# solislemuslab/BayesianNetworkRegression.jl

Hardware: NVIDIA B200
Metric: gibbs_iters_per_sec_all_chains (higher is better)
Workload: dtype f64

## Files before the change

### bayesiannetworkregression.jl_b200/csrc/bnr_linalg.cu

```cuda
#include <cstdio>
#include <cstdlib>
#include <cstring>
#include <cuda.h>
#include "bnr_engine.cuh"
#include "bnr_kernels.h"

namespace bnr {

__device__ __forceinline__ void dmma884(double& c0, double& c1, double a, double b) {
  asm volatile("mma.sync.aligned.m8n8k4.row.col.f64.f64.f64.f64 {%0,%1}, {%2}, {%3}, {%0,%1};\n"
               : "+d"(c0), "+d"(c1) : "d"(a), "d"(b));
}
__device__ __forceinline__ double neg_bits(double x) {
  return __longlong_as_double(__double_as_longlong(x) ^ (long long)0x8000000000000000ull);
}
__device__ __forceinline__ void cp_async_commit() { asm volatile("cp.async.commit_group;\n" ::); }
template <int N>
__device__ __forceinline__ void cp_async_wait() { asm volatile("cp.async.wait_group %0;\n" ::"n"(N)); }
__device__ __forceinline__ void cp_async16(void* smem, const void* gmem) {
  const unsigned sa = (unsigned)__cvta_generic_to_shared(smem);
  asm volatile("cp.async.cg.shared.global [%0], [%1], 16;\n" ::"r"(sa), "l"(gmem));
}

__device__ __forceinline__ unsigned smem_u32(const void* p) { return (unsigned)__cvta_generic_to_shared(p); }
// ... 1297 lines not shown
#pragma unroll
      for (int nf = 0; nf < 4; ++nf) {
        if (nf < nfv) {
#pragma unroll
          for (int mf = 0; mf < 4; ++mf) dmma884(acc[mf][nf][0], acc[mf][nf][1], af[mf], bf[nf]);
        }
      }
    }
  }
  cp_async_wait<0>();
#pragma unroll
  for (int mf = 0; mf < 4; ++mf) {
    const int mm = m0 + wm * 32 + mf * 8 + lr;
#pragma unroll
    for (int nf = 0; nf < 4; ++nf) {
      const int nn = n0 + wn * 32 + nf * 8 + 2 * lk;
      if (mm < M) {
        if (nn < N) o[(size_t)nn * ldout + mm] = acc[mf][nf][0];
        if (nn + 1 < N) o[(size_t)(nn + 1) * ldout + mm] = acc[mf][nf][1];
      }
    }
  }
}

__global__ void k_splitk_reduce(const double* __restrict__ ws, double* __restrict__ out, size_t count, int splits) {
  const size_t i = (size_t)blockIdx.x * blockDim.x + threadIdx.x;
  if (i >= count) return;
  double s = 0.0;
  for (int z = 0; z < splits; ++z) s += ws[(size_t)z * count + i];
  out[i] = s;
}

static int x_times_splits(const Dims& d, int trans) {
  const int M = trans ? d.qp : d.np, K = trans ? d.np : d.qp;
  const int tiles = ((M + XM_BM - 1) / XM_BM) * ((d.C_total + XM_BN - 1) / XM_BN);
  int ks = (2 * 148 + tiles - 1) / tiles;
  const int kmax = K / (4 * XM_BK) > 0 ? K / (4 * XM_BK) : 1;
  if (ks > kmax) ks = kmax;
  if (ks > 64) ks = 64;
  if (ks < 1) ks = 1;
  return ks;
}

size_t x_times_workspace_doubles(const Dims& d) {
  const int a = x_times_splits(d, 0), b = x_times_splits(d, 1);
  const size_t wa = (size_t)a * d.C_total * d.np, wb = (size_t)b * d.C_total * d.qp;
  return wa > wb ? wa : wb;
}

void launch_x_times(const Engine& e, int trans, const double* in, double* out, double* ws, cudaStream_t s) {
  const Dims& d = e.d;
  const int M = trans ? d.qp : d.np, K = trans ? d.np : d.qp, N = d.C;
  const int ldin = trans ? d.np : d.qp, ldout = trans ? d.qp : d.np;
  const int ks = x_times_splits(d, trans);
  const int kper = ((K + ks - 1) / ks + XM_BK - 1) / XM_BK * XM_BK;
  dim3 grid((M + XM_BM - 1) / XM_BM, (N + XM_BN - 1) / XM_BN, ks);
  double* dst = ks == 1 ? out : ws;
  ++g_launches;
  if (trans) k_xmma<1><<<grid, 256, XMMA_SMEM, s>>>(e.X, d.np, M, K, N, in, ldin, dst, ldout, kper);
  else k_xmma<0><<<grid, 256, XMMA_SMEM, s>>>(e.X, d.np, M, K, N, in, ldin, dst, ldout, kper);
  if (ks > 1) {
    const size_t count = (size_t)N * ldout;
    ++g_launches; k_splitk_reduce<<<(unsigned)((count + 255) / 256), 256, 0, s>>>(ws, out, count, ks);
  }
}

__global__ void k_gram_i8(const __grid_constant__ CUtensorMap tmA, const __grid_constant__ CUtensorMap tmB,
                          const double* __restrict__ rscale, double* __restrict__ G, int np, int nvalid, int nkb);
extern const size_t GI_SMEM_BYTES;

void linalg_setup() {
  cudaFuncSetAttribute(k_xmma<0>, cudaFuncAttributeMaxDynamicSharedMemorySize, (int)XMMA_SMEM);
  cudaFuncSetAttribute(k_xmma<1>, cudaFuncAttributeMaxDynamicSharedMemorySize, (int)XMMA_SMEM);
  cudaFuncSetAttribute(k_gram_syrk, cudaFuncAttributeMaxDynamicSharedMemorySize, (int)SYRK_SMEM);
  cudaFuncSetAttribute(k_gram_i8, cudaFuncAttributeMaxDynamicSharedMemorySize, (int)GI_SMEM_BYTES);
  cudaFuncSetAttribute(k_chol_update, cudaFuncAttributeMaxDynamicSharedMemorySize, (int)SYRK_SMEM);
  cudaFuncSetAttribute(k_trsm_dmma, cudaFuncAttributeMaxDynamicSharedMemorySize, (int)SYRK_SMEM);
  cudaFuncSetAttribute(k_potf2_inv, cudaFuncAttributeMaxDynamicSharedMemorySize, (int)POTF2_SMEM);
  cudaFuncSetAttribute(k_bwd_stream, cudaFuncAttributeMaxDynamicSharedMemorySize, 227 * 1024);
  cudaFuncSetAttribute(k_bwd_cluster, cudaFuncAttributeMaxDynamicSharedMemorySize, 227 * 1024);
  cudaFuncSetAttribute(k_small_tile<1, 4>, cudaFuncAttributeMaxDynamicSharedMemorySize, (int)small_tile_smem(32));
  cudaFuncSetAttribute(k_small_tile<2, 4>, cudaFuncAttributeMaxDynamicSharedMemorySize, (int)small_tile_smem(32));
  cudaFuncSetAttribute(k_small_tile<1, 2>, cudaFuncAttributeMaxDynamicSharedMemorySize, (int)small_tile_smem(16));
  cudaFuncSetAttribute(k_small_tile<2, 2>, cudaFuncAttributeMaxDynamicSharedMemorySize, (int)small_tile_smem(16));
  cudaFuncSetAttribute(k_small_tile<1, 8>, cudaFuncAttributeMaxDynamicSharedMemorySize, (int)small_tile_smem(64));
  cudaFuncSetAttribute(k_small_tile<2, 8>, cudaFuncAttributeMaxDynamicSharedMemorySize, (int)small_tile_smem(64));
}

typedef CUresult (*TmapEncodeFn)(CUtensorMap*, CUtensorMapDataType, cuuint32_t, void*, const cuuint64_t*, const cuuint64_t*,
                                 const cuuint32_t*, const cuuint32_t*, CUtensorMapInterleave, CUtensorMapSwizzle,
                                 CUtensorMapL2promotion, CUtensorMapFloatOOBfill);
static TmapEncodeFn g_tmap_encode = nullptr;
bool tmap_setup() {
  if (g_tmap_encode) return true;
  void* fn = nullptr;
  cudaDriverEntryPointQueryResult qr;
  if (cudaGetDriverEntryPoint("cuTensorMapEncodeTiled", &fn, cudaEnableDefault, &qr) != cudaSuccess ||
      qr != cudaDriverEntryPointSuccess || !fn)
    return false;
  g_tmap_encode = (TmapEncodeFn)fn;
  return true;
}
static CUresult encode_map(CUtensorMap* m, const double* base, uint64_t rows, uint64_t krows, uint64_t ld, uint32_t box_rows,
                           uint32_t box_k) {
  memset(m, 0, sizeof(*m));
  const cuuint64_t dims[2] = {rows, krows};
  const cuuint64_t strides[1] = {ld * sizeof(double)};
  const cuuint32_t box[2] = {box_rows, box_k};
  const cuuint32_t estr[2] = {1, 1};
  if (!tmap_setup()) return CUDA_ERROR_NOT_SUPPORTED;
  return g_tmap_encode(m, CU_TENSOR_MAP_DATA_TYPE_FLOAT64, 2, const_cast<double*>(base), dims, strides, box, estr,
                       CU_TENSOR_MAP_INTERLEAVE_NONE, CU_TENSOR_MAP_SWIZZLE_NONE, CU_TENSOR_MAP_L2_PROMOTION_L2_256B,
                       CU_TENSOR_MAP_FLOAT_OOB_FILL_NONE);
}
static CUtensorMap make_map(const double* base, uint64_t rows, uint64_t krows, uint64_t ld, uint32_t box_rows,
                            uint32_t box_k = SY_BK) {
  CUtensorMap m;
  const CUresult r = encode_map(&m, base, rows, krows, ld, box_rows, box_k);
  if (r != CUDA_SUCCESS) {
    fprintf(stderr, "[bnr] cuTensorMapEncodeTiled failed (%d) for a %llu x %llu operand, box %u x %d\n", (int)r,
            (unsigned long long)rows, (unsigned long long)krows, box_rows, (int)box_k);
    abort();
  }
  return m;
}
bool tmaps_check(const Engine& e) {
  const Dims& d = e.d;
  const uint64_t N = d.gdim, C = d.C, T = d.gdim / SY_BT;
  CUtensorMap m;
  bool ok = true;
  if (d.gmode != 2) ok = ok && encode_map(&m, e.X, d.np, d.qp, d.np, SY_LDS, SY_BK) == CUDA_SUCCESS;
  for (uint32_t box : {(uint32_t)SY_LDS, (uint32_t)(SY_BT / 2 + 4), (uint32_t)(SY_BT / 4 + 4)})
    ok = ok && encode_map(&m, e.G, N, N * C, N, box, SY_BK) == CUDA_SUCCESS;
  ok = ok && encode_map(&m, e.Linv, SY_BT, SY_BT * T * C, SY_BT, SY_LDS, SY_BK) == CUDA_SUCCESS;
  ok = ok && encode_map(&m, e.G, N, N * C, N, SY_BT, BW_COLS) == CUDA_SUCCESS;
  ok = ok && encode_map(&m, e.Linv, SY_BT, SY_BT * T * C, SY_BT, SY_BT, BW_COLS) == CUDA_SUCCESS;
  return ok;
}

int syrk_splits(const Dims& d, int C) {
  const int T = d.np / SY_BT, tiles = T * (T + 1) / 2, nk = d.qp / SY_BK;
  if (const char* ov = getenv("BNR_SYRK_SPLITS")) {
    int s = atoi(ov);
    if (s > nk / 8) s = nk / 8;
    return s < 1 ? 1 : (s > SYRK_MAX_SPLITS ? SYRK_MAX_SPLITS : s);
  }
  if (tiles * C >= 148) return 1;
  int s = (4 * 148 + tiles * C - 1) / (tiles * C);
  if (s > nk / 24) s = nk / 24;
  if (s > SYRK_MAX_SPLITS) s = SYRK_MAX_SPLITS;
  return s < 1 ? 1 : s;
}

#ifndef BNR_GI_BK
#define BNR_GI_BK 64
#endif
#ifndef BNR_GI_STAGES
#define BNR_GI_STAGES 2
#endif
constexpr int GI_S = 7;
constexpr int GI_BM = 128, GI_BN = 64;
constexpr int GI_BK = BNR_GI_BK;
constexpr int GI_STAGES = BNR_GI_STAGES;
constexpr int GI_A_PLANE = GI_BM * GI_BK, GI_B_PLANE = GI_BN * GI_BK;
constexpr int GI_STAGE_BYTES = GI_S * (GI_A_PLANE + GI_B_PLANE);
constexpr size_t GI_SMEM = (size_t)GI_STAGES * GI_STAGE_BYTES + 1024 + 256;
const size_t GI_SMEM_BYTES = GI_SMEM;
constexpr int GI_THREADS = 192;
static_assert(GI_BK == 32 || GI_BK == 64 || GI_BK == 128, "k-block = swizzle width");
static_assert(GI_S * GI_BN <= 512, "accumulators exceed tensor memory");

__device__ __forceinline__ unsigned long long gi_desc(unsigned saddr) {
  constexpr unsigned long long layout = GI_BK == 128 ? 2ull : (GI_BK == 64 ? 4ull : 6ull);
  return (unsigned long long)((saddr & 0x3FFFF) >> 4) | (1ull << 16) | ((unsigned long long)((GI_BK * 8) >> 4) << 32) |
         (1ull << 46) | (layout << 61);
}
__host__ __device__ constexpr unsigned gi_idesc(int n) {
  return (2u << 4) | (1u << 7) | (1u << 10) | ((unsigned)(n >> 3) << 17) | ((unsigned)(GI_BM >> 4) << 24);
}

__device__ __forceinline__ void tma_load_3d(void* smem_dst, const CUtensorMap* tm, int x, int y, int z, unsigned long long* bar) {
  asm volatile("cp.async.bulk.tensor.3d.shared::cluster.global.tile.mbarrier::complete_tx::bytes [%0], [%1, {%2, %3, %4}], [%5];\n" ::"r"(
                   smem_u32(smem_dst)), "l"((unsigned long long)tm), "r"(x), "r"(y), "r"(z), "r"(smem_u32(bar)) : "memory");
}
__device__ __forceinline__ void umma_i8(unsigned tmem_d, unsigned long long adesc, unsigned long long bdesc, unsigned idesc,
                                        bool acc) {
  asm volatile("{\n.reg .pred p;\nsetp.ne.b32 p, %4, 0;\ntcgen05.mma.cta_group::1.kind::i8 [%0], %1, %2, %3, p;\n}\n" ::"r"(tmem_d),
               "l"(adesc), "l"(bdesc), "r"(idesc), "r"((int)acc));
}
__device__ __forceinline__ void umma_commit(unsigned long long* bar) {
  asm volatile("tcgen05.commit.cta_group::1.mbarrier::arrive::one.shared::cluster.b64 [%0];\n" ::"r"(smem_u32(bar)) : "memory");
}
__device__ __forceinline__ void tmem_ld8(unsigned taddr, int (&r)[8]) {
  asm volatile("tcgen05.ld.sync.aligned.32x32b.x8.b32 {%0,%1,%2,%3,%4,%5,%6,%7}, [%8];\n"
               : "=r"(r[0]), "=r"(r[1]), "=r"(r[2]), "=r"(r[3]), "=r"(r[4]), "=r"(r[5]), "=r"(r[6]), "=r"(r[7]) : "r"(taddr));
}

constexpr int GS_ROWS = 16, GS_CB = 4, GS_THREADS = 256, GS_TK = 512;
constexpr int GS_TKP = GS_TK + GS_TK / 8;
__device__ __forceinline__ int gs_tidx(int kk) { return kk + 2 * (kk >> 4); }

__device__ __forceinline__ void gs_roots(double (*sq)[GS_TKP], const double* __restrict__ S, int qp, int q, int ncb, int t0) {
  for (int id = threadIdx.x; id < GS_CB * GS_TK; id += GS_THREADS) {
    const int cb = id / GS_TK, kk = id % GS_TK, k = t0 + kk;
    sq[cb][gs_tidx(kk)] = cb < ncb && k < q ? sqrt(S[(size_t)cb * qp + k]) : 0.0;
  }
}

__device__ __forceinline__ void gs_load_x(double (&x)[16], const double* __restrict__ X, int np, int q, int row, int k0) {
  const bool full = k0 + 16 <= q;
#pragma unroll
  for (int j = 0; j < 16; ++j) x[j] = full || k0 + j < q ? X[row + (size_t)np * (k0 + j)] : 0.0;
}

__global__ void __launch_bounds__(GS_THREADS, 2) k_gram_slice(const double* __restrict__ X, const double* __restrict__ S,
                                                            int np, int q, int qp, int C, signed char* __restrict__ planes,
                                                            double* __restrict__ rscale) {
  __shared__ __align__(16) double sq[GS_CB][GS_TKP];
  __shared__ double red[GS_THREADS / 32][GS_CB][GS_ROWS];
  __shared__ double2 scl[GS_CB][GS_ROWS];
  const int lane = threadIdx.x & 31, warp = threadIdx.x >> 5, rr = lane & 15, h = lane >> 4;
  const int r0 = blockIdx.x * GS_ROWS, row = r0 + rr, c0 = blockIdx.y * GS_CB;
  const int ncb = C - c0 < GS_CB ? C - c0 : GS_CB;
  const double* Sb = S + (size_t)c0 * qp;
  constexpr int NW = GS_THREADS / 32, BPW = GS_TK / 32 / NW;
  double x[16];

  double m[GS_CB];
#pragma unroll
  for (int cb = 0; cb < GS_CB; ++cb) m[cb] = 0.0;
  for (int t0 = 0; t0 < q; t0 += GS_TK) {
    __syncthreads();
    gs_roots(sq, Sb, qp, q, ncb, t0);
    __syncthreads();
#pragma unroll
    for (int i = 0; i < BPW; ++i) {
      const int kk = 32 * (warp + NW * i) + 16 * h;
      if (t0 + kk >= q) continue;
      gs_load_x(x, X, np, q, row, t0 + kk);
#pragma unroll
      for (int cb = 0; cb < GS_CB; ++cb) {
        if (cb >= ncb) break;
#pragma unroll
        for (int j = 0; j < 16; j += 2) {
          const double2 s2 = *reinterpret_cast<const double2*>(&sq[cb][gs_tidx(kk + j)]);
          m[cb] = fmax(m[cb], fabs(x[j] * s2.x));
          m[cb] = fmax(m[cb], fabs(x[j + 1] * s2.y));
        }
      }
    }
  }
#pragma unroll
  for (int cb = 0; cb < GS_CB; ++cb) {
    const double o = __shfl_xor_sync(0xffffffffu, m[cb], 16);
    if (h == 0) red[warp][cb][rr] = fmax(m[cb], o);
  }
  __syncthreads();
  if (threadIdx.x < GS_CB * GS_ROWS) {
    const int cb = threadIdx.x / GS_ROWS, i = threadIdx.x % GS_ROWS;
    double mx = 0.0;
#pragma unroll
    for (int w = 0; w < NW; ++w) mx = fmax(mx, red[w][cb][i]);
    int p = 0;
    if (mx > 0.0) {
      p = 54 - ilogb(mx);
      if (ldexp(mx, p) > 126.0 * 0x1p48) --p;
    }
    if (cb < ncb) rscale[(size_t)(c0 + cb) * np + r0 + i] = ldexp(1.0, -p);
    const int p1 = p > 1000 ? 1000 : p;
    scl[cb][i] = make_double2(ldexp(1.0, p1), ldexp(1.0, p - p1));
  }

#if defined(GS_LAB_NO_STORES)
  unsigned sink = 0;
#endif
  for (int t0 = 0; t0 < qp; t0 += GS_TK) {
    __syncthreads();
    gs_roots(sq, Sb, qp, q, ncb, t0);
    __syncthreads();
#pragma unroll 1
    for (int i = 0; i < BPW; ++i) {
      const int kk = 32 * (warp + NW * i) + 16 * h;
      if (t0 + kk >= qp) continue;
      gs_load_x(x, X, np, q, row, t0 + kk);
#pragma unroll 1
      for (int cb = 0; cb < ncb; ++cb) {
        const double2 sc = scl[cb][rr];
        uint4 w[GI_S];
#pragma unroll
        for (int g = 0; g < 4; ++g) {
          unsigned lo[4], hi[4];
#pragma unroll
          for (int b = 0; b < 4; ++b) {
            const int j = 4 * g + b;
#if defined(GS_LAB_NO_DIGITS)
            lo[b] = __double2loint(x[j]) + j; hi[b] = __double2hiint(x[j]) + cb;
#else
            const double sqk = sq[cb][gs_tidx(kk + j)];
            const unsigned long long M = (unsigned long long)__double2ll_rn(x[j] * sqk * sc.x * sc.y) + 0x808080808080ull;
            lo[b] = (unsigned)M; hi[b] = (unsigned)(M >> 32);
#endif
          }
          const unsigned a0 = __byte_perm(lo[0], lo[1], 0x5140), a1 = __byte_perm(lo[0], lo[1], 0x7362);
          const unsigned a2 = __byte_perm(lo[2], lo[3], 0x5140), a3 = __byte_perm(lo[2], lo[3], 0x7362);
          const unsigned b0 = __byte_perm(hi[0], hi[1], 0x5140), b1 = __byte_perm(hi[0], hi[1], 0x7362);
          const unsigned b2 = __byte_perm(hi[2], hi[3], 0x5140), b3 = __byte_perm(hi[2], hi[3], 0x7362);
          const unsigned v[GI_S] = {__byte_perm(b1, b3, 0x5410), __byte_perm(b0, b2, 0x7632) ^ 0x80808080u,
                                    __byte_perm(b0, b2, 0x5410) ^ 0x80808080u, __byte_perm(a1, a3, 0x7632) ^ 0x80808080u,
                                    __byte_perm(a1, a3, 0x5410) ^ 0x80808080u, __byte_perm(a0, a2, 0x7632) ^ 0x80808080u,
                                    __byte_perm(a0, a2, 0x5410) ^ 0x80808080u};
#pragma unroll
          for (int s = 0; s < GI_S; ++s) (&w[s].x)[g] = v[s];
        }
        signed char* out = planes + ((size_t)(c0 + cb) * GI_S * np + row) * qp + t0 + kk;
#pragma unroll
        for (int s = 0; s < GI_S; ++s) {
#if defined(GS_LAB_NO_STORES)
          sink ^= w[s].x ^ w[s].y ^ w[s].z ^ w[s].w;
#else
          *reinterpret_cast<uint4*>(out + (size_t)s * np * qp) = w[s];
#endif
        }
      }
    }
  }
#if defined(GS_LAB_NO_STORES)
  if (sink == 0x9e3779b9u) planes[0] = 1;
#endif
}

__global__ void __launch_bounds__(GI_THREADS, 1)
k_gram_i8(const __grid_constant__ CUtensorMap tmA, const __grid_constant__ CUtensorMap tmB,
          const double* __restrict__ rscale, double* __restrict__ G, int np, int nvalid, int nkb) {
  extern __shared__ __align__(1024) unsigned char gsm_raw[];
  unsigned char* gsm = reinterpret_cast<unsigned char*>(((size_t)gsm_raw + 1023) & ~(size_t)1023);
  unsigned long long* full = reinterpret_cast<unsigned long long*>(gsm + (size_t)GI_STAGES * GI_STAGE_BYTES);
  unsigned long long* empty = full + GI_STAGES;
  unsigned long long* accf = empty + GI_STAGES;
  unsigned* tmem_slot = reinterpret_cast<unsigned*>(accf + 1);
  const int tid = threadIdx.x, lane = tid & 31, warp = tid >> 5;
  const int c = blockIdx.y;
  int ib = 0;
  while (2 * (ib + 1) * (ib + 2) / 2 <= (int)blockIdx.x) ++ib;
  const int jb = (int)blockIdx.x - ib * (ib + 1);
  const int i0 = ib * GI_BM, j0 = jb * GI_BN;
  const bool diag_block = (j0 / GI_BM) == ib;
  int rows_st = GI_BM;
  if (!diag_block) {
    int nfv = (nvalid - i0 + 7) / 8;
    if (nfv <= 0) return;
    rows_st = (nfv < 4 ? 4 : nfv) * 8;
  }
  if (tid == 0) {
    for (int s = 0; s < GI_STAGES; ++s) { mbar_init(&full[s], 1); mbar_init(&empty[s], 1); }
    mbar_init(accf, 1);
    asm volatile("fence.mbarrier_init.release.cluster;\n" ::: "memory");
  }
  if (warp == 0) {
    asm volatile("tcgen05.alloc.cta_group::1.sync.aligned.shared::cta.b32 [%0], 512;\n" ::"r"(smem_u32(tmem_slot)));
    asm volatile("tcgen05.relinquish_alloc_permit.cta_group::1.sync.aligned;\n");
  }
  asm volatile("tcgen05.fence::before_thread_sync;\n" ::: "memory");
  __syncthreads();
  asm volatile("tcgen05.fence::after_thread_sync;\n" ::: "memory");
  const unsigned tmem = *tmem_slot;

  if (warp == 4 && lane == 0) {
#if defined(GI_LAB_MMA_ONLY)
    for (int kb = 0; kb < GI_STAGES && kb < nkb; ++kb) {
#else
    for (int kb = 0; kb < nkb; ++kb) {
#endif
      const int st = kb % GI_STAGES;
      mbar_wait(&empty[st], ((kb / GI_STAGES) & 1) ^ 1);
      unsigned char* sa = gsm + (size_t)st * GI_STAGE_BYTES;
      mbar_expect_tx(&full[st], GI_STAGE_BYTES);
      tma_load_3d(sa, &tmA, kb * GI_BK, i0, c * GI_S, &full[st]);
      tma_load_3d(sa + GI_S * GI_A_PLANE, &tmB, kb * GI_BK, j0, c * GI_S, &full[st]);
    }
  } else if (warp == 5 && lane == 0) {
    for (int kb = 0; kb < nkb; ++kb) {
      const int st = kb % GI_STAGES;
#if defined(GI_LAB_MMA_ONLY)
      if (kb < GI_STAGES) mbar_wait(&full[st], 0);
#else
      mbar_wait(&full[st], (kb / GI_STAGES) & 1);
#endif
      asm volatile("tcgen05.fence::after_thread_sync;\n" ::: "memory");
#if defined(GI_LAB_LOADS_ONLY)
      umma_commit(&empty[st]);
      continue;
#endif
      const unsigned sa = smem_u32(gsm + (size_t)st * GI_STAGE_BYTES), sb = sa + GI_S * GI_A_PLANE;
#pragma unroll
      for (int kk = 0; kk < GI_BK / 32; ++kk) {
#pragma unroll
        for (int s = 0; s < GI_S; ++s) {
          const unsigned long long ad = gi_desc(sa + s * GI_A_PLANE + kk * 32);
#pragma unroll
          for (int t0 = 0; t0 < GI_S - s; t0 += 4) {
            const int nt = GI_S - s - t0 < 4 ? GI_S - s - t0 : 4;
            umma_i8(tmem + (unsigned)((s + t0) * GI_BN), ad, gi_desc(sb + t0 * GI_B_PLANE + kk * 32), gi_idesc(nt * GI_BN),
                    kb > 0 || kk > 0 || s > 0);
          }
        }
      }
      umma_commit(&empty[st]);
    }
    umma_commit(accf);
  } else if (warp < 4) {
    mbar_wait(accf, 0);
    asm volatile("tcgen05.fence::after_thread_sync;\n" ::: "memory");
    const int r = warp * 32 + lane, i = i0 + r;
    const double ri = rscale[(size_t)c * np + i] * 0x1p96;
    double* Gc = G + (size_t)c * np * np;
    const unsigned trow = tmem + ((unsigned)(warp * 32) << 16);
    for (int j8 = 0; j8 < GI_BN; j8 += 8) {
      int acc[GI_S][8];
#pragma unroll
      for (int g = 0; g < GI_S; ++g) tmem_ld8(trow + (unsigned)(g * GI_BN + j8), acc[g]);
      asm volatile("tcgen05.wait::ld.sync.aligned;\n" ::: "memory");
#pragma unroll
      for (int jj = 0; jj < 8; ++jj) {
        const int j = j0 + j8 + jj;
        double v = (double)acc[GI_S - 1][jj];
#pragma unroll
        for (int g = GI_S - 2; g >= 0; --g) v = (double)acc[g][jj] + v * 0x1p-8;
        v = v * ri * rscale[(size_t)c * np + j];
        if (i == j) v += 1.0;
        if (r < rows_st && (i >> 3) >= (j >> 3)) Gc[(size_t)j * np + i] = v;
      }
    }
  }
  asm volatile("tcgen05.fence::before_thread_sync;\n" ::: "memory");
  __syncthreads();
  if (warp == 0) {
    asm volatile("tcgen05.fence::after_thread_sync;\n" ::: "memory");
    asm volatile("tcgen05.dealloc.cta_group::1.sync.aligned.b32 %0, 512;\n" ::"r"(tmem));
  }
}

bool gram_i8_selected(const Dims& d) { return d.gmode == 1 && d.qp >= GRAM_I8_QP_MIN && d.qp <= GRAM_I8_QP_MAX; }

size_t gram_i8_plane_bytes(const Dims& d) { return (size_t)GI_S * d.np * d.qp; }

static CUresult encode_planes_map(CUtensorMap* m, const signed char* planes, const Dims& d, int C, uint32_t box_rows) {
  memset(m, 0, sizeof(*m));
  const cuuint64_t dims[3] = {(cuuint64_t)d.qp, (cuuint64_t)d.np, (cuuint64_t)GI_S * C};
  const cuuint64_t strides[2] = {(cuuint64_t)d.qp, (cuuint64_t)d.qp * d.np};
  const cuuint32_t box[3] = {(cuuint32_t)GI_BK, box_rows, (cuuint32_t)GI_S};
  const cuuint32_t estr[3] = {1, 1, 1};
  const CUtensorMapSwizzle sw = GI_BK == 128 ? CU_TENSOR_MAP_SWIZZLE_128B
                                             : (GI_BK == 64 ? CU_TENSOR_MAP_SWIZZLE_64B : CU_TENSOR_MAP_SWIZZLE_32B);
  if (!tmap_setup()) return CUDA_ERROR_NOT_SUPPORTED;
  return g_tmap_encode(m, CU_TENSOR_MAP_DATA_TYPE_UINT8, 3, const_cast<signed char*>(planes), dims, strides, box, estr,
                       CU_TENSOR_MAP_INTERLEAVE_NONE, sw, CU_TENSOR_MAP_L2_PROMOTION_L2_256B, CU_TENSOR_MAP_FLOAT_OOB_FILL_NONE);
}

static void launch_gram_i8_products(const Engine& e, cudaStream_t s) {
  const Dims& d = e.d;
  CUtensorMap tmA, tmB;
  if (encode_planes_map(&tmA, e.gram_planes, d, d.C, GI_BM) != CUDA_SUCCESS ||
      encode_planes_map(&tmB, e.gram_planes, d, d.C, GI_BN) != CUDA_SUCCESS) {
    fprintf(stderr, "[bnr] cuTensorMapEncodeTiled failed for the Gram digit planes (%d x %d)\n", d.np, d.qp);
    abort();
  }
  const int T = d.np / GI_BM;
  ++g_launches; k_gram_i8<<<dim3(T * (T + 1), d.C), GI_THREADS, GI_SMEM, s>>>(tmA, tmB, e.gram_rscale, e.G, d.np, d.n,
                                                                             (d.qp + GI_BK - 1) / GI_BK);
}

static void launch_gram_slice(const Engine& e, cudaStream_t s) {
  const Dims& d = e.d;
  ++g_launches; k_gram_slice<<<dim3(d.np / GS_ROWS, (d.C + GS_CB - 1) / GS_CB), GS_THREADS, 0, s>>>(
      e.X, e.S, d.np, d.q, d.qp, d.C, e.gram_planes, e.gram_rscale);
}

static void launch_gram_i8(const Engine& e, cudaStream_t s) {
  launch_gram_slice(e, s);
  launch_gram_i8_products(e, s);
}

void launch_syrk_G(const Engine& e, cudaStream_t s) {
  const Dims& d = e.d;
  if (gram_i8_selected(d)) {
    launch_gram_i8(e, s);
    if (e.aux.G_copy) {
      dim3 g2(d.np, d.C);
      ++g_launches; k_copy_sym<<<g2, 256, 0, s>>>(e.G, (size_t)d.np * d.np, d.np, e.aux.G_copy);
    }
    return;
  }
  const int T = d.np / SY_BT;
  const int nk = d.qp / SY_BK;
  const int ns = e.syrk_ws ? e.syrk_ws_cap + 1 : 1;
  const int nk_split = (nk + ns - 1) / ns;
#if defined(SYRK_LAB_ONLY_DIAG)
  dim3 grid(d.C, ns, T);
#elif defined(SYRK_LAB_ONLY_OFFDIAG)
  dim3 grid(d.C, ns, T * (T - 1) / 2);
#else
  dim3 grid(d.C, ns, T * (T + 1) / 2);
#endif
  const size_t gs = (size_t)d.np * d.np;
  const CUtensorMap tmX = make_map(e.X, d.np, d.qp, d.np, SY_LDS);
  ++g_launches; k_gram_syrk<<<grid, SY_THREADS, SYRK_SMEM, s>>>(tmX, e.S, (size_t)d.qp, e.G, gs, d.np, d.n, nk, 1.0,
                                                            nk_split, e.syrk_ws, e.syrk_ws_cap);
  if (ns > 1) {
    dim3 g2(T * (T + 1) / 2 * 8, d.C);
    ++g_launches; k_syrk_splitk_reduce<<<g2, 256, 0, s>>>(e.G, gs, d.np, e.syrk_ws, e.syrk_ws_cap, ns - 1);
  }
  if (e.aux.G_copy) {
    dim3 g2(d.np, d.C);
    ++g_launches; k_copy_sym<<<g2, 256, 0, s>>>(e.G, gs, d.np, e.aux.G_copy);
  }
}

void launch_xtx(const Dims& d, const double* XT, const double* ones, double* XtX, cudaStream_t s) {
  const int T = d.qp / SY_BT;
  dim3 grid(1, 1, T * (T + 1) / 2);
  const CUtensorMap tmXT = make_map(XT, d.qp, d.np, d.qp, SY_LDS);
  ++g_launches; k_gram_syrk<<<grid, SY_THREADS, SYRK_SMEM, s>>>(tmXT, ones, 0, XtX, 0, d.qp, d.q, d.np / SY_BK, 0.0,
                                                            d.np / SY_BK, nullptr, 0);
}

__global__ void __launch_bounds__(256) k_build_P(Engine e) {
  const Dims& d = e.d;
  if (blockIdx.x < blockIdx.y) return;
  const int c = blockIdx.z, N = d.qp;
  const int i = blockIdx.x * 32 + threadIdx.x;
  const double it2 = 1.0 / e.tau2[c];
  double* Gc = e.G + (size_t)c * N * N;
#pragma unroll
  for (int jj = 0; jj < 4; ++jj) {
    const int j = blockIdx.y * 32 + threadIdx.y * 4 + jj;
    if (i < j) continue;
    double v;
    if (i < d.q) {
      v = e.XtX[(size_t)j * N + i] * it2;
      if (i == j) v = (e.XtX[(size_t)j * N + i] + 1.0 / e.S[(size_t)c * d.qp + j]) * it2;
    } else {
      v = (i == j) ? 1.0 : 0.0;
    }
    Gc[(size_t)j * N + i] = v;
  }
}

void launch_build_P(const Engine& e, cudaStream_t s) {
  const Dims& d = e.d;
  dim3 grid(d.qp / 32, d.qp / 32, d.C), block(32, 8);
  ++g_launches; k_build_P<<<grid, block, 0, s>>>(e);
  if (e.aux.G_copy) {
    dim3 g2(d.qp, d.C);
    ++g_launches; k_copy_sym<<<g2, 256, 0, s>>>(e.G, (size_t)d.qp * d.qp, d.qp, e.aux.G_copy);
  }
}

void launch_cholesky(const Engine& e, double* rhs, const ForkJoin& fj, cudaStream_t s) {
  const Dims& d = e.d;
  const int N = d.gdim;
  const int m = d.gmode == 2 ? d.q : d.n;
  const size_t cs = (size_t)N * N;
  const int T = N / PB;
  const size_t ls = (size_t)T * PB * PB;
  static const bool serial = getenv("BNR_CHOL_SERIAL") != nullptr;
  static const int forced = getenv("BNR_CHOL_SCHEDULE") ? atoi(getenv("BNR_CHOL_SCHEDULE")) : 0;
  const bool latency = forced ? forced == 2 : (long long)d.C_total * (T - 1) <= 128;
  ++g_launches; k_augment<<<d.C, 256, 0, s>>>(e.G, cs, N, m, rhs, d.gmode == 2 ? d.qp : d.np, d.gmode == 2 ? e.S : nullptr, e.tau2);
  const CUtensorMap mG = make_map(e.G, N, (uint64_t)N * d.C, N, SY_LDS);
  const CUtensorMap mG2 = make_map(e.G, N, (uint64_t)N * d.C, N, SY_BT / 2 + 4);
  const CUtensorMap mG4 = make_map(e.G, N, (uint64_t)N * d.C, N, SY_BT / 4 + 4);
  const CUtensorMap mL = make_map(e.Linv, PB, (uint64_t)PB * T * d.C, PB, SY_LDS);
  auto mI = [&](int ns) -> const CUtensorMap& { return ns == 4 ? mG4 : (ns == 2 ? mG2 : mG); };

  if (!latency) {
    const bool can_fork = !serial && fj.side != nullptr;
    static const bool a_lo = getenv("BNR_CHOL_A_SIDE_LO") != nullptr;
    cudaStream_t sideA = (!a_lo && fj.side_hi) ? fj.side_hi : fj.side;
    for (int J = 0; J < T; ++J) {
      const bool fork = can_fork && J > 0 && J + 1 < T;
      if (J > 0) {
        const int nk = J * PB / SY_BK;
        if (fork) {
          cudaEventRecord(fj.fork, s);
          cudaStreamWaitEvent(sideA, fj.fork, 0);
          dim3 g2(d.C, T - J - 1);
          ++g_launches; k_chol_update<<<g2, SY_THREADS, SYRK_SMEM, sideA>>>(mG, mG, 0, e.G, cs, N, m + 1, nk, J, J + 1, 1);
          cudaEventRecord(fj.join, sideA);
          dim3 g1(d.C, 1);
          ++g_launches; k_chol_update<<<g1, SY_THREADS, SYRK_SMEM, s>>>(mG, mG, 0, e.G, cs, N, m + 1, nk, J, J, 1);
        } else {
          dim3 g2(d.C, T - J);
          ++g_launches; k_chol_update<<<g2, SY_THREADS, SYRK_SMEM, s>>>(mG, mG, 0, e.G, cs, N, m + 1, nk, J, J, 1);
        }
      }
      ++g_launches; k_potf2_inv<<<d.C, 256, POTF2_SMEM, s>>>(e.G, cs, N, J, e.Linv, T, e.status, 0);
      if (fork) cudaStreamWaitEvent(s, fj.join, 0);
      if (J + 1 < T) {
        dim3 g1(d.C, T - J - 1);
        ++g_launches; k_trsm_dmma<<<g1, SY_THREADS, SYRK_SMEM, s>>>(mL, mG, e.G, cs, N, m + 1, J, J + 1, 1);
      }
    }
    return;
  }

  const bool fork = !serial && fj.side_hi != nullptr && fj.pool != nullptr && fj.npool >= 4 * T;
  cudaStream_t side = fork ? fj.side_hi : s;
  cudaEvent_t* evP = fj.pool;
  cudaEvent_t* evT = fj.pool + T;
  cudaEvent_t* evL = fj.pool + 2 * T;
  cudaEvent_t* evE = fj.pool + 3 * T;
  auto strips = [&](int tiles) {
    static const int fs = getenv("BNR_STRIPS") ? atoi(getenv("BNR_STRIPS")) : 0;
    if (fs == 1 || fs == 2 || fs == 4) return fs;
    const int ctas = d.C_total * tiles;
    return ctas * 4 <= 148 ? 4 : (ctas * 2 <= 148 ? 2 : 1);
// ... 108 lines not shown
```

Before: 11990.

## Split Gram A-tile loads into per-plane barriers and stream digit-plane stores

The Gram int8 product kernel now issues one TMA load and one mbarrier per A digit plane, plus a separate barrier for the whole B block. The MMA warp can then start on plane s as soon as that plane arrives instead of waiting for the full stage. The digit-plane writer in k_gram_slice uses an L2 evict_first cache-hint store with no L1 allocation, so the streamed planes pollute the caches less. In exchange there are more barriers and TMA issues per stage, and the BK and stage compile-time knobs are dropped in favour of fixed constants.

New measurement: 12470, median of 6. 4.1% higher.

```diff
diff --git a/bayesiannetworkregression.jl_b200/csrc/bnr_linalg.cu b/bayesiannetworkregression.jl_b200/csrc/bnr_linalg.cu
--- a/bayesiannetworkregression.jl_b200/csrc/bnr_linalg.cu
+++ b/bayesiannetworkregression.jl_b200/csrc/bnr_linalg.cu
@@ -1473,28 +1473,27 @@
   return s < 1 ? 1 : s;
 }
 
-#ifndef BNR_GI_BK
-#define BNR_GI_BK 64
-#endif
-#ifndef BNR_GI_STAGES
-#define BNR_GI_STAGES 2
-#endif
 constexpr int GI_S = 7;
 constexpr int GI_BM = 128, GI_BN = 64;
-constexpr int GI_BK = BNR_GI_BK;
-constexpr int GI_STAGES = BNR_GI_STAGES;
-constexpr int GI_A_PLANE = GI_BM * GI_BK, GI_B_PLANE = GI_BN * GI_BK;
-constexpr int GI_STAGE_BYTES = GI_S * (GI_A_PLANE + GI_B_PLANE);
-constexpr size_t GI_SMEM = (size_t)GI_STAGES * GI_STAGE_BYTES + 1024 + 256;
+constexpr int GI_BK = 64;
+constexpr int GI_STAGES = 2;
+constexpr int GI_A_PLANE = GI_BM * GI_BK, GI_B_PLANE = GI_BN * GI_BK, GI_B_BLOCK = GI_S * GI_B_PLANE;
+constexpr int GI_STAGE_BYTES = GI_S * GI_A_PLANE + GI_B_BLOCK;
+constexpr size_t GI_SMEM = (size_t)GI_STAGES * GI_STAGE_BYTES + 1024 + 512;
 const size_t GI_SMEM_BYTES = GI_SMEM;
 constexpr int GI_THREADS = 192;
-static_assert(GI_BK == 32 || GI_BK == 64 || GI_BK == 128, "k-block = swizzle width");
 static_assert(GI_S * GI_BN <= 512, "accumulators exceed tensor memory");
+static_assert(GI_STAGES * (GI_S + 2) * 8 + 8 + 4 <= 512, "barriers exceed their space");
+static_assert(GI_SMEM + 23552 + 2 * 1024 <= 228 * 1024, "k_gram_i8 would no longer leave room for a k_gram_slice CTA");
+#if defined(GI_LAB_MMA_ONLY)
+constexpr bool GI_FILL_ONCE = true;
+#else
+constexpr bool GI_FILL_ONCE = false;
+#endif
 
 __device__ __forceinline__ unsigned long long gi_desc(unsigned saddr) {
-  constexpr unsigned long long layout = GI_BK == 128 ? 2ull : (GI_BK == 64 ? 4ull : 6ull);
   return (unsigned long long)((saddr & 0x3FFFF) >> 4) | (1ull << 16) | ((unsigned long long)((GI_BK * 8) >> 4) << 32) |
-         (1ull << 46) | (layout << 61);
+         (1ull << 46) | (4ull << 61);
 }
 __host__ __device__ constexpr unsigned gi_idesc(int n) {
   return (2u << 4) | (1u << 7) | (1u << 10) | ((unsigned)(n >> 3) << 17) | ((unsigned)(GI_BM >> 4) << 24);
@@ -1520,6 +1519,16 @@
 constexpr int GS_ROWS = 16, GS_CB = 4, GS_THREADS = 256, GS_TK = 512;
 constexpr int GS_TKP = GS_TK + GS_TK / 8;
 __device__ __forceinline__ int gs_tidx(int kk) { return kk + 2 * (kk >> 4); }
+
+__device__ __forceinline__ unsigned long long gs_policy_stream() {
+  unsigned long long p;
+  asm("createpolicy.fractional.L2::evict_first.b64 %0, 1.0;\n" : "=l"(p));
+  return p;
+}
+__device__ __forceinline__ void gs_st16(void* p, uint4 w, unsigned long long pol) {
+  asm volatile("st.global.L1::no_allocate.L2::cache_hint.v4.u32 [%0], {%1, %2, %3, %4}, %5;\n" ::"l"(p), "r"(w.x), "r"(w.y),
+               "r"(w.z), "r"(w.w), "l"(pol) : "memory");
+}
 
 __device__ __forceinline__ void gs_roots(double (*sq)[GS_TKP], const double* __restrict__ S, int qp, int q, int ncb, int t0) {
   for (int id = threadIdx.x; id < GS_CB * GS_TK; id += GS_THREADS) {
@@ -1545,6 +1554,7 @@
   const int ncb = C - c0 < GS_CB ? C - c0 : GS_CB;
   const double* Sb = S + (size_t)c0 * qp;
   constexpr int NW = GS_THREADS / 32, BPW = GS_TK / 32 / NW;
+  const unsigned long long stream = gs_policy_stream();
   double x[16];
 
   double m[GS_CB];
@@ -1639,7 +1649,7 @@
 #if defined(GS_LAB_NO_STORES)
           sink ^= w[s].x ^ w[s].y ^ w[s].z ^ w[s].w;
 #else
-          *reinterpret_cast<uint4*>(out + (size_t)s * np * qp) = w[s];
+          gs_st16(out + (size_t)s * np * qp, w[s], stream);
 #endif
         }
       }
@@ -1655,8 +1665,9 @@
           const double* __restrict__ rscale, double* __restrict__ G, int np, int nvalid, int nkb) {
   extern __shared__ __align__(1024) unsigned char gsm_raw[];
   unsigned char* gsm = reinterpret_cast<unsigned char*>(((size_t)gsm_raw + 1023) & ~(size_t)1023);
-  unsigned long long* full = reinterpret_cast<unsigned long long*>(gsm + (size_t)GI_STAGES * GI_STAGE_BYTES);
-  unsigned long long* empty = full + GI_STAGES;
+  unsigned long long* afull = reinterpret_cast<unsigned long long*>(gsm + (size_t)GI_STAGES * GI_STAGE_BYTES);
+  unsigned long long* bfull = afull + GI_STAGES * GI_S;
+  unsigned long long* empty = bfull + GI_STAGES;
   unsigned long long* accf = empty + GI_STAGES;
   unsigned* tmem_slot = reinterpret_cast<unsigned*>(accf + 1);
   const int tid = threadIdx.x, lane = tid & 31, warp = tid >> 5;
@@ -1673,7 +1684,8 @@
     rows_st = (nfv < 4 ? 4 : nfv) * 8;
   }
   if (tid == 0) {
-    for (int s = 0; s < GI_STAGES; ++s) { mbar_init(&full[s], 1); mbar_init(&empty[s], 1); }
+    for (int s = 0; s < GI_STAGES * GI_S; ++s) mbar_init(&afull[s], 1);
+    for (int s = 0; s < GI_STAGES; ++s) { mbar_init(&bfull[s], 1); mbar_init(&empty[s], 1); }
     mbar_init(accf, 1);
     asm volatile("fence.mbarrier_init.release.cluster;\n" ::: "memory");
   }
@@ -1687,36 +1699,33 @@
   const unsigned tmem = *tmem_slot;
 
   if (warp == 4 && lane == 0) {
-#if defined(GI_LAB_MMA_ONLY)
-    for (int kb = 0; kb < GI_STAGES && kb < nkb; ++kb) {
-#else
-    for (int kb = 0; kb < nkb; ++kb) {
-#endif
+    for (int kb = 0; kb < nkb && (!GI_FILL_ONCE || kb < GI_STAGES); ++kb) {
       const int st = kb % GI_STAGES;
       mbar_wait(&empty[st], ((kb / GI_STAGES) & 1) ^ 1);
       unsigned char* sa = gsm + (size_t)st * GI_STAGE_BYTES;
-      mbar_expect_tx(&full[st], GI_STAGE_BYTES);
-      tma_load_3d(sa, &tmA, kb * GI_BK, i0, c * GI_S, &full[st]);
-      tma_load_3d(sa + GI_S * GI_A_PLANE, &tmB, kb * GI_BK, j0, c * GI_S, &full[st]);
+      mbar_expect_tx(&bfull[st], GI_B_BLOCK);
+      tma_load_3d(sa + GI_S * GI_A_PLANE, &tmB, kb * GI_BK, j0, c * GI_S, &bfull[st]);
+      for (int s = 0; s < GI_S; ++s) {
+        mbar_expect_tx(&afull[st * GI_S + s], GI_A_PLANE);
+        tma_load_3d(sa + s * GI_A_PLANE, &tmA, kb * GI_BK, i0, c * GI_S + s, &afull[st * GI_S + s]);
+      }
     }
   } else if (warp == 5 && lane == 0) {
     for (int kb = 0; kb < nkb; ++kb) {
       const int st = kb % GI_STAGES;
-#if defined(GI_LAB_MMA_ONLY)
-      if (kb < GI_STAGES) mbar_wait(&full[st], 0);
-#else
-      mbar_wait(&full[st], (kb / GI_STAGES) & 1);
-#endif
-      asm volatile("tcgen05.fence::after_thread_sync;\n" ::: "memory");
-#if defined(GI_LAB_LOADS_ONLY)
-      umma_commit(&empty[st]);
-      continue;
-#endif
+      const unsigned ph = (kb / GI_STAGES) & 1;
+      const bool wait = !GI_FILL_ONCE || kb < GI_STAGES;
+      if (wait) mbar_wait(&bfull[st], ph);
       const unsigned sa = smem_u32(gsm + (size_t)st * GI_STAGE_BYTES), sb = sa + GI_S * GI_A_PLANE;
 #pragma unroll
       for (int kk = 0; kk < GI_BK / 32; ++kk) {
 #pragma unroll
         for (int s = 0; s < GI_S; ++s) {
+          if (kk == 0) {
+            if (wait) mbar_wait(&afull[st * GI_S + s], ph);
+            asm volatile("tcgen05.fence::after_thread_sync;\n" ::: "memory");
+          }
+#if !defined(GI_LAB_LOADS_ONLY)
           const unsigned long long ad = gi_desc(sa + s * GI_A_PLANE + kk * 32);
 #pragma unroll
           for (int t0 = 0; t0 < GI_S - s; t0 += 4) {
@@ -1724,6 +1733,7 @@
             umma_i8(tmem + (unsigned)((s + t0) * GI_BN), ad, gi_desc(sb + t0 * GI_B_PLANE + kk * 32), gi_idesc(nt * GI_BN),
                     kb > 0 || kk > 0 || s > 0);
           }
+#endif
         }
       }
       umma_commit(&empty[st]);
@@ -1765,24 +1775,23 @@
 
 size_t gram_i8_plane_bytes(const Dims& d) { return (size_t)GI_S * d.np * d.qp; }
 
-static CUresult encode_planes_map(CUtensorMap* m, const signed char* planes, const Dims& d, int C, uint32_t box_rows) {
+static CUresult encode_planes_map(CUtensorMap* m, const signed char* planes, const Dims& d, int C, uint32_t box_rows,
+                                  uint32_t box_planes) {
   memset(m, 0, sizeof(*m));
   const cuuint64_t dims[3] = {(cuuint64_t)d.qp, (cuuint64_t)d.np, (cuuint64_t)GI_S * C};
   const cuuint64_t strides[2] = {(cuuint64_t)d.qp, (cuuint64_t)d.qp * d.np};
-  const cuuint32_t box[3] = {(cuuint32_t)GI_BK, box_rows, (cuuint32_t)GI_S};
+  const cuuint32_t box[3] = {(cuuint32_t)GI_BK, box_rows, box_planes};
   const cuuint32_t estr[3] = {1, 1, 1};
-  const CUtensorMapSwizzle sw = GI_BK == 128 ? CU_TENSOR_MAP_SWIZZLE_128B
-                                             : (GI_BK == 64 ? CU_TENSOR_MAP_SWIZZLE_64B : CU_TENSOR_MAP_SWIZZLE_32B);
   if (!tmap_setup()) return CUDA_ERROR_NOT_SUPPORTED;
   return g_tmap_encode(m, CU_TENSOR_MAP_DATA_TYPE_UINT8, 3, const_cast<signed char*>(planes), dims, strides, box, estr,
-                       CU_TENSOR_MAP_INTERLEAVE_NONE, sw, CU_TENSOR_MAP_L2_PROMOTION_L2_256B, CU_TENSOR_MAP_FLOAT_OOB_FILL_NONE);
+                       CU_TENSOR_MAP_INTERLEAVE_NONE, CU_TENSOR_MAP_SWIZZLE_64B, CU_TENSOR_MAP_L2_PROMOTION_L2_256B, CU_TENSOR_MAP_FLOAT_OOB_FILL_NONE);
 }
 
 static void launch_gram_i8_products(const Engine& e, cudaStream_t s) {
   const Dims& d = e.d;
   CUtensorMap tmA, tmB;
-  if (encode_planes_map(&tmA, e.gram_planes, d, d.C, GI_BM) != CUDA_SUCCESS ||
-      encode_planes_map(&tmB, e.gram_planes, d, d.C, GI_BN) != CUDA_SUCCESS) {
+  if (encode_planes_map(&tmA, e.gram_planes, d, d.C, GI_BM, 1) != CUDA_SUCCESS ||
+      encode_planes_map(&tmB, e.gram_planes, d, d.C, GI_BN, GI_S) != CUDA_SUCCESS) {
     fprintf(stderr, "[bnr] cuTensorMapEncodeTiled failed for the Gram digit planes (%d x %d)\n", d.np, d.qp);
     abort();
   }
```

## Remap gram-slice lanes, double column block, add prefetch and streaming stores

Applied to the files above, without the earlier changes.

Restructures k_gram_slice so each lane owns one (row, 16-wide k chunk) per tile: the column block grows from 4 to 8 and the k tile shrinks from 512 to 256. The max reduction now uses intra-8-lane shuffles instead of per-warp shared arrays. It also prefetches the next tile of X into L1 and writes the int8 planes with streaming (__stcs) stores so they do not pollute cache. The aim is to reuse each X load across more columns and to cut memory latency and cache pressure. The risks are more registers from m[8], lower parallelism in the grid's y dimension, and prefetches that may be wasted.

Result: faster. 11860 before, 12150 after (median of 6 runs) (+2.4%).

```diff
diff --git a/bayesiannetworkregression.jl_b200/csrc/bnr_linalg.cu b/bayesiannetworkregression.jl_b200/csrc/bnr_linalg.cu
--- a/bayesiannetworkregression.jl_b200/csrc/bnr_linalg.cu
+++ b/bayesiannetworkregression.jl_b200/csrc/bnr_linalg.cu
@@ -1517,8 +1517,9 @@
                : "=r"(r[0]), "=r"(r[1]), "=r"(r[2]), "=r"(r[3]), "=r"(r[4]), "=r"(r[5]), "=r"(r[6]), "=r"(r[7]) : "r"(taddr));
 }
 
-constexpr int GS_ROWS = 16, GS_CB = 4, GS_THREADS = 256, GS_TK = 512;
+constexpr int GS_ROWS = 16, GS_CB = 8, GS_THREADS = 256, GS_TK = 256;
 constexpr int GS_TKP = GS_TK + GS_TK / 8;
+static_assert(GS_ROWS == 4 * (GS_THREADS / 32 / 2) && GS_TK == 2 * 8 * 16, "lane -> (row, k) map of k_gram_slice");
 __device__ __forceinline__ int gs_tidx(int kk) { return kk + 2 * (kk >> 4); }
 
 __device__ __forceinline__ void gs_roots(double (*sq)[GS_TKP], const double* __restrict__ S, int qp, int q, int ncb, int t0) {
@@ -1528,60 +1529,97 @@
   }
 }
 
-__device__ __forceinline__ void gs_load_x(double (&x)[16], const double* __restrict__ X, int np, int q, int row, int k0) {
+__device__ __forceinline__ unsigned long long gs_x_policy() {
+  unsigned long long pol;
+  asm("createpolicy.fractional.L2::evict_last.b64 %0, 1.0;" : "=l"(pol));
+  return pol;
+}
+__device__ __forceinline__ double gs_ld_x(const double* p, unsigned long long pol) {
+#if defined(GS_LAB_HINTS) && (GS_LAB_HINTS & 1)
+  double v;
+  asm("ld.global.nc.L2::cache_hint.f64 %0, [%1], %2;" : "=d"(v) : "l"(p), "l"(pol));
+  return v;
+#else
+  return *p;
+#endif
+}
+__device__ __forceinline__ void gs_st_plane(signed char* p, uint4 v) {
+#if defined(GS_LAB_HINTS) && !(GS_LAB_HINTS & 2)
+  *reinterpret_cast<uint4*>(p) = v;
+#else
+  __stcs(reinterpret_cast<uint4*>(p), v);
+#endif
+}
+
+__device__ __forceinline__ void gs_load_x(double (&x)[16], const double* __restrict__ X, int np, int q, int row, int k0,
+                                          unsigned long long pol) {
   const bool full = k0 + 16 <= q;
 #pragma unroll
-  for (int j = 0; j < 16; ++j) x[j] = full || k0 + j < q ? X[row + (size_t)np * (k0 + j)] : 0.0;
+  for (int j = 0; j < 16; ++j) x[j] = full || k0 + j < q ? gs_ld_x(X + row + (size_t)np * (k0 + j), pol) : 0.0;
+}
+
+__device__ __forceinline__ void gs_prefetch_x(const double* __restrict__ X, int np, int q, int row, int k0) {
+#if !defined(GS_LAB_NO_PREFETCH)
+#pragma unroll
+  for (int j = 0; j < 16; ++j)
+    if (k0 + j < q) {
+#if defined(GS_LAB_PREFETCH_L2)
+      asm volatile("prefetch.global.L2 [%0];" ::"l"(X + row + (size_t)np * (k0 + j)));
+#else
+      asm volatile("prefetch.global.L1 [%0];" ::"l"(X + row + (size_t)np * (k0 + j)));
+#endif
+    }
+#endif
 }
 
 __global__ void __launch_bounds__(GS_THREADS, 2) k_gram_slice(const double* __restrict__ X, const double* __restrict__ S,
                                                             int np, int q, int qp, int C, signed char* __restrict__ planes,
                                                             double* __restrict__ rscale) {
   __shared__ __align__(16) double sq[GS_CB][GS_TKP];
-  __shared__ double red[GS_THREADS / 32][GS_CB][GS_ROWS];
+  __shared__ double red[2][GS_CB][GS_ROWS];
   __shared__ double2 scl[GS_CB][GS_ROWS];
-  const int lane = threadIdx.x & 31, warp = threadIdx.x >> 5, rr = lane & 15, h = lane >> 4;
+  const int lane = threadIdx.x & 31, warp = threadIdx.x >> 5, rr = 4 * (warp & 3) + (lane >> 3), h = warp >> 2;
+  const int kk = 128 * h + 16 * (lane & 7);
   const int r0 = blockIdx.x * GS_ROWS, row = r0 + rr, c0 = blockIdx.y * GS_CB;
   const int ncb = C - c0 < GS_CB ? C - c0 : GS_CB;
   const double* Sb = S + (size_t)c0 * qp;
-  constexpr int NW = GS_THREADS / 32, BPW = GS_TK / 32 / NW;
+  const unsigned long long xpol = gs_x_policy();
   double x[16];
 
   double m[GS_CB];
 #pragma unroll
   for (int cb = 0; cb < GS_CB; ++cb) m[cb] = 0.0;
+#if !defined(GS_LAB_CONST_STORES)
   for (int t0 = 0; t0 < q; t0 += GS_TK) {
     __syncthreads();
     gs_roots(sq, Sb, qp, q, ncb, t0);
     __syncthreads();
-#pragma unroll
-    for (int i = 0; i < BPW; ++i) {
-      const int kk = 32 * (warp + NW * i) + 16 * h;
-      if (t0 + kk >= q) continue;
-      gs_load_x(x, X, np, q, row, t0 + kk);
-#pragma unroll
-      for (int cb = 0; cb < GS_CB; ++cb) {
-        if (cb >= ncb) break;
-#pragma unroll
-        for (int j = 0; j < 16; j += 2) {
-          const double2 s2 = *reinterpret_cast<const double2*>(&sq[cb][gs_tidx(kk + j)]);
-          m[cb] = fmax(m[cb], fabs(x[j] * s2.x));
-          m[cb] = fmax(m[cb], fabs(x[j + 1] * s2.y));
-        }
-      }
-    }
-  }
+    if (t0 + kk >= q) continue;
+    gs_load_x(x, X, np, q, row, t0 + kk, xpol);
+    gs_prefetch_x(X, np, q, row, (t0 + GS_TK < q ? t0 + GS_TK : 0) + kk);
+#pragma unroll
+    for (int cb = 0; cb < GS_CB; ++cb) {
+      if (cb >= ncb) break;
+#pragma unroll
+      for (int j = 0; j < 16; j += 2) {
+        const double2 s2 = *reinterpret_cast<const double2*>(&sq[cb][gs_tidx(kk + j)]);
+        m[cb] = fmax(m[cb], fabs(x[j] * s2.x));
+        m[cb] = fmax(m[cb], fabs(x[j + 1] * s2.y));
+      }
+    }
+  }
+#endif
 #pragma unroll
   for (int cb = 0; cb < GS_CB; ++cb) {
-    const double o = __shfl_xor_sync(0xffffffffu, m[cb], 16);
-    if (h == 0) red[warp][cb][rr] = fmax(m[cb], o);
+    m[cb] = fmax(m[cb], __shfl_xor_sync(0xffffffffu, m[cb], 1));
+    m[cb] = fmax(m[cb], __shfl_xor_sync(0xffffffffu, m[cb], 2));
+    m[cb] = fmax(m[cb], __shfl_xor_sync(0xffffffffu, m[cb], 4));
+    if ((lane & 7) == 0) red[h][cb][rr] = m[cb];
   }
   __syncthreads();
   if (threadIdx.x < GS_CB * GS_ROWS) {
     const int cb = threadIdx.x / GS_ROWS, i = threadIdx.x % GS_ROWS;
-    double mx = 0.0;
-#pragma unroll
-    for (int w = 0; w < NW; ++w) mx = fmax(mx, red[w][cb][i]);
+    const double mx = fmax(red[0][cb][i], red[1][cb][i]);
     int p = 0;
     if (mx > 0.0) {
       p = 54 - ilogb(mx);
@@ -1597,51 +1635,57 @@
 #endif
   for (int t0 = 0; t0 < qp; t0 += GS_TK) {
     __syncthreads();
+#if !defined(GS_LAB_CONST_STORES)
     gs_roots(sq, Sb, qp, q, ncb, t0);
+#endif
     __syncthreads();
+    if (t0 + kk >= qp) continue;
+#if !defined(GS_LAB_CONST_STORES)
+    gs_load_x(x, X, np, q, row, t0 + kk, xpol);
+    gs_prefetch_x(X, np, q, row, t0 + GS_TK + kk);
+#endif
 #pragma unroll 1
-    for (int i = 0; i < BPW; ++i) {
-      const int kk = 32 * (warp + NW * i) + 16 * h;
-      if (t0 + kk >= qp) continue;
-      gs_load_x(x, X, np, q, row, t0 + kk);
-#pragma unroll 1
-      for (int cb = 0; cb < ncb; ++cb) {
-        const double2 sc = scl[cb][rr];
-        uint4 w[GI_S];
-#pragma unroll
-        for (int g = 0; g < 4; ++g) {
-          unsigned lo[4], hi[4];
-#pragma unroll
-          for (int b = 0; b < 4; ++b) {
-            const int j = 4 * g + b;
+    for (int cb = 0; cb < ncb; ++cb) {
+      const double2 sc = scl[cb][rr];
+      uint4 w[GI_S];
+#if defined(GS_LAB_CONST_STORES)
+#pragma unroll
+      for (int s = 0; s < GI_S; ++s) w[s] = make_uint4(s, cb, t0, kk);
+#else
+#pragma unroll
+      for (int g = 0; g < 4; ++g) {
+        unsigned lo[4], hi[4];
+#pragma unroll
+        for (int b = 0; b < 4; ++b) {
+          const int j = 4 * g + b;
 #if defined(GS_LAB_NO_DIGITS)
-            lo[b] = __double2loint(x[j]) + j; hi[b] = __double2hiint(x[j]) + cb;
+          lo[b] = __double2loint(x[j]) + j; hi[b] = __double2hiint(x[j]) + cb;
 #else
-            const double sqk = sq[cb][gs_tidx(kk + j)];
-            const unsigned long long M = (unsigned long long)__double2ll_rn(x[j] * sqk * sc.x * sc.y) + 0x808080808080ull;
-            lo[b] = (unsigned)M; hi[b] = (unsigned)(M >> 32);
-#endif
-          }
-          const unsigned a0 = __byte_perm(lo[0], lo[1], 0x5140), a1 = __byte_perm(lo[0], lo[1], 0x7362);
-          const unsigned a2 = __byte_perm(lo[2], lo[3], 0x5140), a3 = __byte_perm(lo[2], lo[3], 0x7362);
-          const unsigned b0 = __byte_perm(hi[0], hi[1], 0x5140), b1 = __byte_perm(hi[0], hi[1], 0x7362);
-          const unsigned b2 = __byte_perm(hi[2], hi[3], 0x5140), b3 = __byte_perm(hi[2], hi[3], 0x7362);
-          const unsigned v[GI_S] = {__byte_perm(b1, b3, 0x5410), __byte_perm(b0, b2, 0x7632) ^ 0x80808080u,
-                                    __byte_perm(b0, b2, 0x5410) ^ 0x80808080u, __byte_perm(a1, a3, 0x7632) ^ 0x80808080u,
-                                    __byte_perm(a1, a3, 0x5410) ^ 0x80808080u, __byte_perm(a0, a2, 0x7632) ^ 0x80808080u,
-                                    __byte_perm(a0, a2, 0x5410) ^ 0x80808080u};
-#pragma unroll
-          for (int s = 0; s < GI_S; ++s) (&w[s].x)[g] = v[s];
+          const double sqk = sq[cb][gs_tidx(kk + j)];
+          const unsigned long long M = (unsigned long long)__double2ll_rn(x[j] * sqk * sc.x * sc.y) + 0x808080808080ull;
+          lo[b] = (unsigned)M; hi[b] = (unsigned)(M >> 32);
+#endif
         }
-        signed char* out = planes + ((size_t)(c0 + cb) * GI_S * np + row) * qp + t0 + kk;
-#pragma unroll
-        for (int s = 0; s < GI_S; ++s) {
+        const unsigned a0 = __byte_perm(lo[0], lo[1], 0x5140), a1 = __byte_perm(lo[0], lo[1], 0x7362);
+        const unsigned a2 = __byte_perm(lo[2], lo[3], 0x5140), a3 = __byte_perm(lo[2], lo[3], 0x7362);
+        const unsigned b0 = __byte_perm(hi[0], hi[1], 0x5140), b1 = __byte_perm(hi[0], hi[1], 0x7362);
+        const unsigned b2 = __byte_perm(hi[2], hi[3], 0x5140), b3 = __byte_perm(hi[2], hi[3], 0x7362);
+        const unsigned v[GI_S] = {__byte_perm(b1, b3, 0x5410), __byte_perm(b0, b2, 0x7632) ^ 0x80808080u,
+                                  __byte_perm(b0, b2, 0x5410) ^ 0x80808080u, __byte_perm(a1, a3, 0x7632) ^ 0x80808080u,
+                                  __byte_perm(a1, a3, 0x5410) ^ 0x80808080u, __byte_perm(a0, a2, 0x7632) ^ 0x80808080u,
+                                  __byte_perm(a0, a2, 0x5410) ^ 0x80808080u};
+#pragma unroll
+        for (int s = 0; s < GI_S; ++s) (&w[s].x)[g] = v[s];
+      }
+#endif
+      signed char* out = planes + ((size_t)(c0 + cb) * GI_S * np + row) * qp + t0 + kk;
+#pragma unroll
+      for (int s = 0; s < GI_S; ++s) {
 #if defined(GS_LAB_NO_STORES)
-          sink ^= w[s].x ^ w[s].y ^ w[s].z ^ w[s].w;
+        sink ^= w[s].x ^ w[s].y ^ w[s].z ^ w[s].w;
 #else
-          *reinterpret_cast<uint4*>(out + (size_t)s * np * qp) = w[s];
-#endif
-        }
+        gs_st_plane(out + (size_t)s * np * qp, w[s]);
+#endif
       }
     }
   }
```
